# lucabaldesi/srsRAN

Hardware: AMD Instinct MI355X
Metric: PDSCH decoded Mbps + code-blocks/sec, 20 MHz TM4 QAM256, 1/2/4/8 GPU (higher is better)
Workload: dtype fp32+int16; 1 GPU; srslte_ue_dl chain from time-domain I/Q: 2048 subframes/GPU/batch, 20 MHz (100 PRB), TM4 2x2 spatial multiplexing, 2 codewords QAM256 TBS 97896 (C=16, K=6144), MMSE+CSI, max 10 half-its with CRC early stop, 40 dB crossed 2x2 channel, every subframe distinct (GPU eNodeB generator, keyed by global subframe index); 3 PHY worker threads (own ue_dl / stream / softbuffers each) decode alternate batches,; subframes_per_gpu_batch=2048, code_blocks_per_gpu_batch=65536, workers_per_gpu=3, parallelism=dp1

## Files before the change

### srsran_amd/csrc/dlsch_internal.h

```cpp
#pragma once
#include <hip/hip_runtime.h>
#include <stdint.h>

#define SB_STRIDE 18600
#define SB_DATA 768
#define SB_CONV8 10240
#define SB_ROWMASK 18544
#define SB_ROWMASK_WORDS 12

namespace mi355 {

struct CbDesc {
  uint32_t tb, cb, C;
  uint32_t rlen;
  uint32_t rp, n_e;
  uint32_t rv;
  uint32_t slot;
  uint64_t e_off;
  uint64_t data_off;
};

struct TbDesc {
  uint32_t tbs, C, C1, K1, K2, slot0, invalid;
  uint32_t Qm, nof_e_bits, rv;
// ... 98 lines not shown
```

### srsran_amd/csrc/dlsch_runtime.cpp

```cpp
#include <hip/hip_runtime.h>

#include <algorithm>
#include <chrono>
#include <stdlib.h>
#include <map>
#include <mutex>
#include <stdio.h>
#include <string.h>
#include <vector>

#include "../../include/srsran_amd/dlsch.h"
#include "../../include/srsran_amd/tdec.h"
#include "device_mem.h"
#include "dlsch_internal.h"
#include "host_staging.h"
#include "tdec8_internal.h"
#include "rm_image.h"
#include "rm_tables.h"
#include "runtime_internal.h"
#include "tdec_internal.h"

using namespace mi355;

struct mi355_softbuffer_pool {
  int      device = 0;
  uint32_t nof_sb = 0, max_cb = 0;
  int16_t* buf    = nullptr;
  uint8_t* cb_crc = nullptr;
  uint8_t* data   = nullptr;
  uint8_t* fresh  = nullptr;
  mi355::DevMem d_list[2];
  uint32_t   list_cap[2] = {0, 0};
  hipEvent_t ev_list[2]  = {nullptr, nullptr};
  bool       ev_armed[2] = {false, false};
  uint32_t   lpar        = 0;
  mi355::HostStaging st_list;
};

CrcTable mi355::make_crc_table(uint32_t poly)
{
  CrcTable t{};
  t.poly = poly;
  for (uint32_t i = 0; i < 256; i++) {
    uint32_t c = i << 16;
    for (int j = 0; j < 8; j++) c = (c & 0x800000) ? ((c << 1) ^ poly) & 0xffffff : (c << 1) & 0xffffff;
// ... 81 lines not shown
  return old;
}

static bool spec_enabled()
{
  static const bool on = !getenv("MI355_TDEC_SPEC") || atoi(getenv("MI355_TDEC_SPEC")) != 0;
  return on;
}

static bool no_rowmask()
{
  static const bool off = getenv("MI355_NO_ROWMASK") && atoi(getenv("MI355_NO_ROWMASK")) != 0;
  return off;
}

static bool lat_waves4()
{
  static const bool on = getenv("MI355_LAT_WAVES") && atoi(getenv("MI355_LAT_WAVES")) == 4;
  return on;
}
static bool lat_owaves()
{
  static const bool on = !getenv("MI355_LAT_OWAVES") || atoi(getenv("MI355_LAT_OWAVES")) != 0;
  return on;
}

bool mi355::rm_sparse_writes()
{
  static const bool on = !getenv("MI355_RM_SPARSE") || atoi(getenv("MI355_RM_SPARSE")) != 0;
  return on && !no_rowmask();
// ... 116 lines not shown
extern "C" {

int mi355_softbuffer_pool_create(mi355_softbuffer_pool_t** p, uint32_t nof_sb, uint32_t max_cb, int device)
{
  if (!p || !nof_sb || !max_cb) return MI355_ERROR_INVALID_INPUTS;
  CHECK_HIP(hipSetDevice(device));
  auto*        s  = new mi355_softbuffer_pool;
  const size_t nc = (size_t)nof_sb * max_cb;
  s->device       = device;
  s->nof_sb       = nof_sb;
  s->max_cb       = max_cb;
  if (hipMalloc(&s->buf, nc * SB_STRIDE * 2) != hipSuccess || hipMalloc(&s->cb_crc, nc) != hipSuccess ||
      hipMalloc(&s->data, nc * SB_DATA) != hipSuccess || hipMalloc(&s->fresh, nc) != hipSuccess) {
    mi355_softbuffer_pool_destroy(s);
    return MI355_ERROR;
  }
  (void)hipMemset(s->fresh, 1, nc);
  (void)hipMemset(s->cb_crc, 0, nc);
  (void)hipMemset(s->data, 0, nc * SB_DATA);
  (void)hipDeviceSynchronize();
  *p = s;
  return MI355_SUCCESS;
}

void mi355_softbuffer_pool_destroy(mi355_softbuffer_pool_t* p)
{
  if (!p) return;
  (void)hipFree(p->buf);
  (void)hipFree(p->cb_crc);
  (void)hipFree(p->data);
// ... 305 lines not shown
    }
    memcpy(all.data() + off, qlist.data(), qlist.size() * 4);
    CHECK_HIP(ent.d.upload(all));
    ent.nq = (uint32_t)qlist.size(), ent.qoff = off;
    return MI355_SUCCESS;
  });
  if (e) return e;
  *tab  = c->d.as<uint16_t>();
  *nq   = c->nq;
  *qoff = c->qoff;
  return MI355_SUCCESS;
}

mi355::SoftbufferView mi355::softbuffer_view(mi355_softbuffer_pool_t* p)
{
  return SoftbufferView{p->buf, SB_STRIDE, p->cb_crc, p->fresh, p->nof_sb, p->max_cb};
}

int mi355::dlsch_decode_dev_hook(mi355_dlsch_t* q, mi355_softbuffer_pool_t* pool, const void* d_e_bits,
                                 const mi355_dlsch_tb_t* tbs, uint32_t ntb, uint8_t* d_data, int32_t* ret,
                                 float* avg_iterations, void* stream, mi355::WaitHook hook, bool llr8,
                                 mi355::DlschPending* pend, bool after_s, bool rm_done)
{
  if (!q || !pool || !tbs || !ret || (ntb && !d_e_bits)) return MI355_ERROR_INVALID_INPUTS;
  if (ntb == 0) return MI355_SUCCESS;
  std::lock_guard<std::mutex> lock(q->mu);
  static const bool prof = getenv("MI355_HOST_PROF") != nullptr;
  auto              now  = [] { return std::chrono::steady_clock::now(); };
  const auto        t0   = now();
  CHECK_HIP(hipSetDevice(q->device));
  hipStream_t s = stream ? (hipStream_t)stream : q->own;

  std::vector<TbDesc>                        tbd(ntb);
  std::vector<std::pair<uint32_t, uint32_t>> kcount;
  std::vector<uint32_t>                      rvmask;
  std::vector<uint32_t>                      fold2;
  auto group_of = [&](uint32_t K) {
// ... 227 lines not shown
      if (lat[li]) continue;
      if (lv.t8) {
        T8Batch b{};
        b.in = (int8_t*)pool->buf, b.in_stride = SB_STRIDE * sizeof(int16_t), b.slot = d_slot + lv.off;
        b.done = d_done + lv.off, b.running = d_run + h, b.K = lv.K, b.ncb = lv.n;
        if ((r = tdec8_halfit_batch(lv.t8, b, h, lv.dec, lv.K / 8, s))) return r;
      }
      DlschCheckArgs ca{d_cb + lv.off, (int)lv.n, lv.K, h, q->max_its, lv.dec, lv.K / 8, d_data,
                        d_done + lv.off, d_run + h, d_run + h + 1, d_its + lv.off, pool->cb_crc, &crc[0], &crc[1],
                        lv.scale};
      bool fused = false;
      if (!lv.t8) {
        TdecRun rq{llr8 ? pool->buf + SB_CONV8 : pool->buf, SB_STRIDE, d_slot + lv.off, d_done + lv.off, d_run + h, lv.n,
                   lv.K, h, h + 1, lv.dec, lv.K / 8, s, &ca, &fused};
        rq.rowmask = !llr8 && !no_rowmask();
        bool taken = false;
        rq.spec       = spec;
        rq.spec_taken = &taken;
        if ((r = mi355_tdec_run_internal(lv.td, rq))) return r;
        if (!fused) CHECK_HIP(dlsch_launch_check(ca, s));
        if (taken && h + 1 < q->max_its) {
          TdecRun rd = rq;
          rd.remaining  = d_run + h + 1;
          rd.chk        = nullptr;
          rd.chk_fused  = nullptr;
          rd.spec       = false;
          rd.spec_taken = nullptr;
          rd.redo       = true;
          if ((r = mi355_tdec_run_internal(lv.td, rd))) return r;
        }
// ... 52 lines not shown
```

### srsran_amd/csrc/pdsch_internal.h

```cpp
#pragma once
#include <hip/hip_runtime.h>
#include <stdint.h>

namespace mi355 {

constexpr uint32_t EQ_BLOCK_ITEMS = 1024;

constexpr uint32_t PDSCH_GOLD_MAX = 14u * 12u * 110u * 8u;

struct PdschJobDev {
  const float2*   y[2];
  const float2*   h[4][2];
  const uint16_t* map;
  const uint16_t* imap;
  uint32_t        g0;
  float2*         d[2];
  float*          csi[2];
  uint32_t*       cmax;
  uint32_t        cmax_stride;
  uint32_t        nof_re, nof_rx, nof_ports, nof_layers, scheme, cb;
  uint32_t        row;
  uint32_t        row_magic;
  uint32_t        h_invariant;
  uint32_t        rhob_mask;
// ... 40 lines not shown
};
struct EqRmJob {
  uint32_t  C, Qm, Gp;
  EqRmLayer layer[2];
  const uint16_t* cmp[2][2];
  uint32_t        cnq[2][2], cqoff[2][2];
};
struct EqRmPool {
  int16_t*       sb;
  size_t         sb_stride;
  const uint8_t* sb_crc;
  uint8_t*       fresh;
  int            sparse;
  int            diag = 0;
  unsigned long long* prof = nullptr;
};
hipError_t pdsch_launch_eq_rm(const PdschJobDev* jobs, const EqRmJob* rj, uint32_t njobs, uint32_t max_c, uint32_t img,
                              uint32_t cimg, const uint32_t* keys, uint32_t nkeys, const EqRmPool& pool, hipStream_t s);

}
```

### srsran_amd/csrc/pdsch_kernels.hip

```cpp
#include <hip/hip_runtime.h>

#include <algorithm>
#include <stdint.h>

#include "pdsch_internal.h"
#include "rm_image.h"
#include "xcd.h"

namespace mi355 {

namespace {

struct cf {
  float re, im;
};
__device__ __forceinline__ cf mk(float r, float i) { return cf{r, i}; }
__device__ __forceinline__ cf operator+(cf a, cf b) { return mk(a.re + b.re, a.im + b.im); }
__device__ __forceinline__ cf operator-(cf a, cf b) { return mk(a.re - b.re, a.im - b.im); }
__device__ __forceinline__ cf operator*(cf a, cf b) { return mk(a.re * b.re - a.im * b.im, a.re * b.im + a.im * b.re); }
__device__ __forceinline__ cf operator*(cf a, float s) { return mk(a.re * s, a.im * s); }
__device__ __forceinline__ cf cj(cf a) { return mk(a.re, -a.im); }
__device__ __forceinline__ cf mulj(cf a) { return mk(-a.im, a.re); }
__device__ __forceinline__ float abs2(cf a) { return a.re * a.re + a.im * a.im; }
#define GLB __attribute__((address_space(1)))
// ... 1127 lines not shown
  static_assert(ER_THREADS >= 128 && 2 * (2 * SB_ROWMASK_WORDS + 1) <= 64, "pdsch_eq_rm prologue waves");
  if (tid - 64 < 2 && J.cw[tid - 64]) {
    const uint32_t l = tid - 64;
    cwd[l]           = *J.cw[l];
    cmb[l]           = cwd[l].csi_enable ? *gptr(cwd[l].cmax_final) : 0u;
  }
  __syncthreads();
  const uint32_t kx0 = c < R.layer[0].C1 ? 0u : 1u, kx1 = c < R.layer[1].C1 ? 0u : 1u;
  const bool     lean = need[0] && need[1] && fresh[0] && fresh[1] && R.layer[0].inv[kx0] == R.layer[1].inv[kx1] &&
                    R.layer[0].buflen[kx0] == R.layer[1].buflen[kx1];
  const uint32_t ev = c > R.C - gamma ? 1u : 0u;
  const bool     cm = lean && P.sparse && QM0 == QM1 && R.cmp[kx0][ev] != nullptr;
  const GLB uint16_t* fw  = cm ? gptr(R.cmp[kx0][ev]) : nullptr;
  const uint32_t      cnq = cm ? R.cnq[kx0][ev] : 0u;
  uint32_t* const     im32 = (uint32_t*)imgs;
  const unsigned long long pt1 = P.prof ? clock64() : 0ull;
  const float         noise = J.noise_dev ? *gptr(J.noise_dev) : J.noise;
  const uint32_t      row = J.row, magic = J.row_magic, rmask = J.rhob_mask;
  const float         rinv = J.rhob_inv;
  const GLB float2*   yp[2] = {gptr(J.y[0]), gptr(J.nof_rx > 1 ? J.y[1] : J.y[0])};
  const GLB float2*   hp[4];
  h_ptrs(J, hp);
  const GLB fv4*      wtp = (const GLB fv4*)gptr(J.wtab);
  uint4 iv0[ER_Q];
  if constexpr (ER_TPF) {
    if (lean) {
      const uint32_t  npairs = R.layer[0].buflen[kx0] / 2;
      const GLB uint32_t* inv32 = (const GLB uint32_t*)gptr(R.layer[0].inv[kx0]);
#pragma unroll
      for (int k = 0; k < ER_Q; k++) {
// ... 141 lines not shown
          for (int p = 0; p < 8; p++) w[p] = (m >> p) & 1u ? w[p] : 0u;
          const uint4    v0 = make_uint4(__builtin_amdgcn_perm(w[1], w[0], 0x05040100u), __builtin_amdgcn_perm(w[3], w[2], 0x05040100u),
                                         __builtin_amdgcn_perm(w[5], w[4], 0x05040100u), __builtin_amdgcn_perm(w[7], w[6], 0x05040100u));
          const uint4    v1 = make_uint4(__builtin_amdgcn_perm(w[1], w[0], 0x07060302u), __builtin_amdgcn_perm(w[3], w[2], 0x07060302u),
                                         __builtin_amdgcn_perm(w[5], w[4], 0x07060302u), __builtin_amdgcn_perm(w[7], w[6], 0x07060302u));
          const uint32_t i  = 4 * (qd[k] & 0xffffu);
          if (al && i + 3 < npairs) {
            __builtin_nontemporal_store((u4v){v0.x, v0.y, v0.z, v0.w}, (GLB u4v*)(sb[0] + i));
            __builtin_nontemporal_store((u4v){v1.x, v1.y, v1.z, v1.w}, (GLB u4v*)(sb[1] + i));
          } else {
            const uint32_t a0[4] = {v0.x, v0.y, v0.z, v0.w}, a1[4] = {v1.x, v1.y, v1.z, v1.w};
#pragma unroll
            for (int cc = 0; cc < 4; cc++)
              if (i + cc < npairs) sb[0][i + cc] = a0[cc], sb[1][i + cc] = a1[cc];
          }
        }
      }
      need[0] = need[1] = false;
    } else if (lean) {
      const uint32_t  npairs = R.layer[0].buflen[kx0] / 2, Kc = (R.layer[0].N[kx0] - 12) / 3;
      const GLB uint32_t* inv32 = (const GLB uint32_t*)gptr(R.layer[0].inv[kx0]);
      GLB uint32_t*   sb[2]  = {(GLB uint32_t*)gptr(P.sb + (size_t)slot[0] * P.sb_stride),
                                (GLB uint32_t*)gptr(P.sb + (size_t)slot[1] * P.sb_stride)};
      const bool      al     = (((uintptr_t)sb[0] | (uintptr_t)sb[1]) & 15) == 0;
      const uint16_t* a0     = (const uint16_t*)imgs;
      const uint16_t* a1     = (const uint16_t*)(imgs + img);
#pragma unroll 1
      for (int rd = 0; rd < ER_R; rd++) {
        uint4 iv[ER_Q];
#pragma unroll
        for (int k = 0; k < ER_Q; k++) {
// ... 241 lines not shown
```

### srsran_amd/csrc/pdsch_runtime.cpp

```cpp
#include <hip/hip_runtime.h>

#include <algorithm>
#include <chrono>
#include <stdlib.h>
#include <cmath>
#include <map>
#include <unordered_map>
#include <atomic>
#include <mutex>
#include <stdio.h>
#include <string.h>
#include <string>
#include <vector>

#include "../../include/srsran_amd/dlsch.h"
#include "../../include/srsran_amd/pdsch.h"
#include "../../include/srsran_amd/tdec.h"
#include "device_mem.h"
#include "host_staging.h"
#include "lte_common.h"
#include "pdsch_internal.h"
#include "rm_tables.h"
#include "runtime_internal.h"

// ... 756 lines not shown
        }
      }
    }
    if (nt < 2) {
      for (auto& row : R.cmp) row[0] = row[1] = nullptr;
    } else {
      er.cimg = std::max(er.cimg, cimg);
    }
    er.max_c = std::max(er.max_c, nt ? R.C : 0u);
    er.img   = std::max(er.img, n_max);
  }
  er.pool = EqRmPool{v.buf, v.stride, v.cb_crc, v.fresh, rm_sparse_writes() ? 1 : 0};
  static const int eqrm_diag = getenv("MI355_EQRM_DIAG") ? atoi(getenv("MI355_EQRM_DIAG")) : 0;
  er.pool.diag = eqrm_diag;
  er.pool.prof = g_eqrm_prof.load();
  return er.max_c > 0;
}

int mi355::pdsch_decode_batch_dev_noise(mi355_pdsch_t* q, mi355_softbuffer_pool_t* pool, const mi355_pdsch_job_t* jobs,
                                        uint32_t njobs, mi355_pdsch_res_t* res, void* stream, const float* d_noise,
                                        WaitHook hook, bool ce_invariant, PdschPending* pend, bool after_s)
{
  if (!q || !pool || !res || (njobs && !jobs)) return MI355_ERROR_INVALID_INPUTS;
  std::lock_guard<std::mutex> lock(q->mu);
  static const bool prof = getenv("MI355_HOST_PROF") != nullptr;
  auto              now  = [] { return std::chrono::steady_clock::now(); };
  const auto        t0   = now();
  CHECK_HIP(hipSetDevice(q->device));
  hipStream_t          s = stream ? (hipStream_t)stream : q->own;
  std::vector<JobPlan> plans(njobs);
// ... 51 lines not shown
      const uint32_t g = pend->used;
      if (pend->groups.size() <= g) {
        pend->groups.emplace_back(new DlschPending);
        pend->ret.emplace_back();
        pend->avg.emplace_back();
        pend->who.emplace_back();
      }
      dp = pend->groups[g].get(), ret = &pend->ret[g], avg = &pend->avg[g];
      pend->who[g] = by_its[its];
    }
    ret->assign(kv.second.size(), 0);
    avg->assign(kv.second.size(), 0.f);
    if ((r = mi355_dlsch_set_max_iterations(q->dlsch, its))) return r;
    const bool after = after_s || (pend && pend->used > 0);
    r = dlsch_decode_dev_hook(q->dlsch, pool, q->e_arena, kv.second.data(), (uint32_t)kv.second.size(), nullptr,
                              ret->data(), avg->data(), s, hook, q->llr8, dp, after, eqrm);
    hook = WaitHook{};
    if (r) return r;
    if (pend)
      pend->used++;
    else
      fill_results(res, by_its[its], *ret, *avg);
  }
  return MI355_SUCCESS;
}

int mi355::PdschPending::collect()
{
  int r = MI355_SUCCESS;
  for (uint32_t g = 0; g < used; g++) {
    const int e = groups[g]->collect();
// ... 12 lines not shown
```

### srsran_amd/csrc/runtime_internal.h

```cpp
#pragma once
#include "../../include/srsran_amd/dlsch.h"
#include "../../include/srsran_amd/pdsch.h"

#include <hip/hip_runtime.h>

#include <memory>
#include <utility>
#include <atomic>
#include <vector>

namespace mi355 {

struct WaitHook {
  void (*fn)(void*) = nullptr;
  void* ctx         = nullptr;
};

struct DlschPending {
  char*                host = nullptr;
  size_t               cap  = 0;
  hipEvent_t           ev   = nullptr;
  bool                 armed = false;
  uint32_t             ntb   = 0;
  size_t               avg_off = 0;
  std::vector<uint8_t> invalid;
  int32_t*             ret = nullptr;
  float*               avg = nullptr;
  std::atomic<uint32_t>* spec_mask = nullptr;
  uint32_t             max_its   = 0;
  DlschPending()                    = default;
  DlschPending(const DlschPending&) = delete;
  ~DlschPending();
  int collect();
};

int dlsch_decode_dev_hook(mi355_dlsch_t* q, mi355_softbuffer_pool_t* pool, const void* d_e_bits,
                          const mi355_dlsch_tb_t* tbs, uint32_t ntb, uint8_t* d_data, int32_t* ret, float* avg_iterations,
                          void* stream, WaitHook hook, bool llr8 = false, DlschPending* pend = nullptr,
                          bool after_s = false, bool rm_done = false);

int      dlsch_rm_inv(mi355_dlsch_t* q, uint32_t K, uint32_t rv, const uint16_t** out);
uint32_t dlsch_rm_buflen(uint32_t K);
int      dlsch_rm_compact(mi355_dlsch_t* q, uint32_t K, uint32_t rv, uint32_t E, const uint16_t** tab, uint32_t* nq,
                          uint32_t* qoff);
bool     rm_sparse_writes();
struct SoftbufferView {
  int16_t* buf;
  size_t   stride;
  uint8_t* cb_crc;
  uint8_t* fresh;
  uint32_t nof_sb, max_cb;
};
SoftbufferView softbuffer_view(mi355_softbuffer_pool_t* p);

struct PdschPending {
  std::vector<std::unique_ptr<DlschPending>>                   groups;
  std::vector<std::vector<int32_t>>                            ret;
  std::vector<std::vector<float>>                              avg;
  std::vector<std::vector<std::pair<uint32_t, uint32_t>>>      who;
  uint32_t                                                     used = 0;
  mi355_pdsch_res_t*                                           res  = nullptr;
  int collect();
};

int pdsch_decode_batch_dev_noise(mi355_pdsch_t* q, mi355_softbuffer_pool_t* pool, const mi355_pdsch_job_t* jobs,
                                 uint32_t njobs, mi355_pdsch_res_t* res, void* stream, const float* d_noise,
// ... 5 lines not shown
```

### srsran_amd/csrc/tdec_internal.h

```cpp
#pragma once
#include <hip/hip_runtime.h>
#include <stdint.h>

#include "dlsch_internal.h"

#define TDEC_INF 10000
#define TDEC_WARMUP 40
#define TDEC_SEG 8

namespace mi355 {

struct TdecWinArgs {
  const int16_t*  in;
  size_t          in_stride;
  const uint32_t* in_idx;
  const uint8_t*  done;
  const uint32_t* remaining;
  uint32_t*       A1;
  uint32_t*       E;
  uint32_t*       D;
  uint32_t*       ckpt;
  const uint32_t* dstE;
  const uint32_t* dstA;
  int             ncb, L, Lp, nseg, n, write_d;
  uint8_t*        dec;
  size_t          dec_stride;
  const uint32_t* gS;
  const uint32_t* gP;
  DlschCheckArgs  chk;
  int             chk_on;
  int             spec;
  int             rowmask;
};

struct TdecDecideArgs {
  const uint32_t* D;
  uint8_t*        out;
  size_t          out_stride;
  int             ncb, L, Lp;
  const uint8_t*  done;
  const uint32_t* remaining;
};

struct TdecGenArgs {
  const uint32_t* S;
  const uint32_t* P0;
  const uint32_t* P1;
// ... 57 lines not shown
  const int16_t*  in;
  size_t          in_stride;
  const uint32_t* in_idx;
  const uint8_t*  done;
  const uint32_t* remaining;
  uint32_t        n, K, h0, h1;
  uint8_t*        out;
  size_t          out_stride;
  hipStream_t     stream;
  const DlschCheckArgs* chk = nullptr;
  bool*                 chk_fused = nullptr;
  bool  spec       = false;
  bool* spec_taken = nullptr;
  bool  redo       = false;
  bool  rowmask    = false;
};

hipError_t tdec_win_launch_halfit(int nsb, const TdecWinArgs& a, hipStream_t s);
bool       tdec_win_spec_ok(int nsb, int L);
int        tdec_set_diag(int mode);
hipError_t tdec_win_launch_decide(int nsb, const TdecDecideArgs& a, hipStream_t s);
hipError_t tdec_gen_launch_prep(const TdecGenPrepArgs& a, hipStream_t s);
hipError_t tdec_gen_launch_halfit(const TdecGenArgs& a, hipStream_t s);
hipError_t tdec_gen_launch_decide(const TdecGenDecideArgs& a, hipStream_t s);

}

struct mi355_tdec_batch;
int mi355_tdec_run_internal(mi355_tdec_batch* q, const mi355::TdecRun& r);
int mi355_tdec_win_tables(mi355_tdec_batch* q, uint32_t K, const uint32_t** dstE, const uint32_t** dstA);
// ... 1 lines not shown
```

### srsran_amd/csrc/tdec_kernels.hip

```cpp
#include <hip/hip_runtime.h>

#include <atomic>
#include <stdint.h>
#include <stdlib.h>

#include "crc_device.h"
#include "tdec_internal.h"

namespace mi355 {

typedef short v2s __attribute__((ext_vector_type(2)));

__device__ __forceinline__ v2s U(uint32_t u) { return __builtin_bit_cast(v2s, u); }
__device__ __forceinline__ uint32_t W(v2s v) { return __builtin_bit_cast(uint32_t, v); }
__device__ __forceinline__ v2s sadd(v2s a, v2s b) { return __builtin_elementwise_add_sat(a, b); }
__device__ __forceinline__ v2s ssub(v2s a, v2s b) { return __builtin_elementwise_sub_sat(a, b); }
__device__ __forceinline__ v2s vmax(v2s a, v2s b) { return __builtin_elementwise_max(a, b); }
__device__ __forceinline__ v2s splat(short s) { return (v2s){s, s}; }
__device__ __forceinline__ uint32_t hi_lo(uint32_t a, uint32_t b) { return __builtin_amdgcn_alignbit(b, a, 16); }
__device__ __forceinline__ uint32_t from_prev(uint32_t v)
{
  return (uint32_t)__builtin_amdgcn_update_dpp(0, (int)v, 0x111, 0xf, 0xf, true);
}
__device__ __forceinline__ uint32_t from_next(uint32_t v)
// ... 110 lines not shown
      } else {
        c.done[cb] = 2;
      }
    }
  }
  const uint64_t un = __builtin_amdgcn_ballot_w64(l == 0 && !fin);
  if (un && (threadIdx.x & 63) == (uint32_t)__builtin_ctzll(un)) flag_set(c.next);
}


#define WG_AT(arr, j) (arr)[((size_t)grp * Lp + (j)) * 64 + q]

#define TDEC_BM_WORDS (8 * 193)
__shared__ uint32_t tdec_tx_lds[4][2][TDEC_SEG * 64];
__shared__ uint32_t tdec_ym_lds[4][8 * SB_ROWMASK_WORDS];
__shared__ uint32_t tdec_bm_lds[4 * TDEC_BM_WORDS];
__shared__ int16_t  tdec_stg_lds[4][TDEC_SEG * 128];
__shared__ uint32_t tdec_stg_row[4][TDEC_SEG];

#ifndef TDEC_WAVES_PER_EU
#define TDEC_WAVES_PER_EU 2
#endif
#ifndef TDEC_NPH
#define TDEC_NPH 1
#endif
#ifndef TDEC_FPF
#define TDEC_FPF 2
#endif
#ifndef TDEC_CLONE_NO_E
#define TDEC_CLONE_NO_E 0
// ... 19 lines not shown
#ifndef TDEC_OUT_AUX
#define TDEC_OUT_AUX -1
#endif
#ifndef TDEC_CK_AUX
#define TDEC_CK_AUX -1
#endif
#ifndef TDEC_CLONE_NO_FIN
#define TDEC_CLONE_NO_FIN 0
#endif
#ifndef TDEC_CLONE_NO_TAB
#define TDEC_CLONE_NO_TAB 0
#endif
#ifndef TDEC_CLONE_CK_HALF
#define TDEC_CLONE_CK_HALF 0
#endif
template <int NSB, int SEG, int MODE, int DIAG, bool FULL, int OUTK, bool GI = false, bool TX = false>
__device__ __forceinline__ void tdec_win_body(const TdecWinArgs& a, const int gl,
                                              const uint32_t (*crc_t4)[4][256] = nullptr)
{
  constexpr int NL = NSB / 2;
  constexpr int G  = 64 / NL;
  static_assert(!TX || (NSB == 16 && FULL && SEG == 8), "TX loads need 8-lane rows and whole 8-step segments");
  const int     grp = __builtin_amdgcn_readfirstlane(gl >> 6), q = gl & 63;
  const int     cbg = q / NL, l = q % NL;
  if constexpr (!TX) {
    if (grp * G + cbg >= a.ncb) return;
    if (a.done && a.done[grp * G + cbg]) return;
  }
  if (a.remaining && *a.remaining == 0) return;

  const int  L = a.L, Lp = a.Lp, nseg = a.nseg;
  constexpr bool CL     = DIAG == 20;
  constexpr bool dec2   = MODE == 2;
  constexpr bool has_ap = MODE == 1;

  const int       cb   = grp * G + cbg;
  const int       K    = L * NSB;
// ... 22 lines not shown
  }
  constexpr bool RMK = NSB == 16 && !GI;
  uint32_t*      ymask = nullptr;
  if constexpr (RMK) {
    ymask = tdec_ym_lds[threadIdx.x >> 6];
#pragma unroll
    for (int w = l; w < SB_ROWMASK_WORDS; w += NL) {
      uint32_t v = 0xffffffffu;
      if (a.rowmask) v = ((const uint32_t*)(a.in + bidx * a.in_stride + SB_ROWMASK))[(dec2 ? SB_ROWMASK_WORDS : 0) + w];
      ymask[cbg * SB_ROWMASK_WORDS + w] = v;
    }
    __builtin_amdgcn_fence(__ATOMIC_RELEASE, "wavefront");
    __builtin_amdgcn_wave_barrier();
    __builtin_amdgcn_fence(__ATOMIC_ACQUIRE, "wavefront");
  }
  auto yrow = [&](int c, int j) -> bool {
    if constexpr (RMK) {
      return (ymask[c * SB_ROWMASK_WORDS + (j >> 5)] >> (j & 31)) & 1u;
    } else {
      return true;
    }
  };
  auto tx_load = [&](int so, int j0, uint32_t* r, bool par = false) {
    uint4 v0 = make_uint4(0u, 0u, 0u, 0u), v1 = v0;
    const int tc = (q >> 1) & 7, jr = j0 + (q >> 4);
    if (!par || yrow(tc, jr)) v0 = txin[so + j0 * 2];
    if (!par || yrow(tc, jr + 4)) v1 = txin[so + (j0 + 4) * 2];
    r[0] = v0.x; r[1] = v0.y; r[2] = v0.z; r[3] = v0.w;
    r[4] = v1.x; r[5] = v1.y; r[6] = v1.z; r[7] = v1.w;
  };
  auto tx_unpack = [&](int b, const uint32_t* r, uint32_t* o) {
    uint32_t* w = txb + b * SEG * 64;
    ((uint4*)w)[q]      = make_uint4(r[0], r[1], r[2], r[3]);
    ((uint4*)w)[64 + q] = make_uint4(r[4], r[5], r[6], r[7]);
    __builtin_amdgcn_fence(__ATOMIC_RELEASE, "wavefront");
    __builtin_amdgcn_wave_barrier();
    __builtin_amdgcn_fence(__ATOMIC_ACQUIRE, "wavefront");
#pragma unroll
    for (int i = 0; i < SEG; i++) o[i] = w[64 * i + q];
  };

  v2s st[8], nw[8], aw[8];

  set_minf(aw);
#pragma unroll 1
  for (int b = 0; b < TDEC_WARMUP / 8; b++) {
    uint32_t xo[8], yo[8], ao[8] = {};
#pragma unroll
    for (int i = 0; i < 8; i++) {
      const int j = (L - TDEC_WARMUP) + 8 * b + i;
      xo[i]       = X[j * xs];
      yo[i]       = yrow(cbg, j) ? Y[j * ys] : 0u;
      if constexpr (has_ap) ao[i] = AP[j * 64];
    }
#pragma unroll
    for (int i = 0; i < 8; i++) {
      const int k = 8 * b + i;
      v2s       x = U(hi_lo(from_prev(xo[i]), xo[i]));
      if constexpr (has_ap) x = sadd(x, U(hi_lo(from_prev(ao[i]), ao[i])));
      if constexpr (CL) {
        aw[k & 7] = aw[k & 7] ^ x ^ U(yo[i]);
        continue;
      }
      v2s c0[8], c1[8];
      alpha_cands<true>(aw, x, U(hi_lo(from_prev(yo[i]), yo[i])), c0, c1);
#pragma unroll
      for (int s = 0; s < 8; s++) aw[s] = vmax(c0[s], c1[s]);
      if ((k & 1) == 0 && k != 0) normalize<true>(aw);
    }
  }

  if constexpr (DIAG != 2) {
  set_minf(st);
#pragma unroll 1
  for (int b = TDEC_WARMUP / 8 - 1; b >= 0; b--) {
    uint32_t xo[8], yo[8], ao[8] = {};
#pragma unroll
    for (int i = 0; i < 8; i++) {
      const int j = 8 * b + i;
      xo[i]       = X[j * xs];
      yo[i]       = yrow(cbg, j) ? Y[j * ys] : 0u;
      if constexpr (has_ap) ao[i] = AP[j * 64];
    }
#pragma unroll
    for (int i = 7; i >= 0; i--) {
      const int k = 8 * b + i;
      v2s       x = U(hi_lo(xo[i], from_next(xo[i])));
      if constexpr (has_ap) x = sadd(x, U(hi_lo(ao[i], from_next(ao[i]))));
      if constexpr (CL) {
        st[k & 7] = st[k & 7] ^ x ^ U(yo[i]);
        continue;
      }
      beta_step<true>(st, x, U(hi_lo(yo[i], from_next(yo[i]))), nw);
#pragma unroll
      for (int s = 0; s < 8; s++) st[s] = nw[s];
      if ((k & 1) == 0 && k != 0) normalize<true>(st);
// ... 22 lines not shown
      ck[((size_t)(nseg - 1) * 8 + s) * 64] = W(st[s]);
    }
  }

  {
    uint32_t cx[SEG], cy[SEG], ca[SEG] = {};
    auto     load = [&](int t, uint32_t* x, uint32_t* y, uint32_t* ap) {
      if constexpr (TX) {
        if constexpr (!dec2) tx_load(txoX, t * SEG, x);
        tx_load(txoY, t * SEG, y, true);
      }
#pragma unroll
      for (int i = 0; i < SEG; i++) {
        const int j = FULL ? t * SEG + i : min(t * SEG + i, L - 1);
        if constexpr (!TX || dec2) x[i] = X[j * xs];
        if constexpr (!TX) y[i] = yrow(cbg, j) ? Y[j * ys] : 0u;
        if constexpr (has_ap) ap[i] = AP[j * 64];
      }
    };
    uint32_t bx[SEG], by[SEG], ba[SEG] = {}, dx[SEG], dy[SEG], da[SEG] = {};
    load(nseg - 1, cx, cy, ca);
    if (nseg > 1) load(nseg - 2, bx, by, ba);
    auto seg = [&](int t, const uint32_t* rx, const uint32_t* ry, const uint32_t* sa, uint32_t* lx, uint32_t* ly,
                   uint32_t* la) {
      uint32_t sx[SEG], sy[SEG];
      if constexpr (TX) {
        if constexpr (!dec2) tx_unpack(0, rx, sx);
        tx_unpack(1, ry, sy);
      }
#pragma unroll
      for (int i = 0; i < SEG; i++) {
// ... 134 lines not shown
  };
  uint32_t cx[SEG], cy[SEG], ca[SEG] = {}, cd[SEG], cc[8];
  constexpr bool NFIN = CL && TDEC_CLONE_NO_FIN, NTAB = CL && TDEC_CLONE_NO_TAB, NCK = CL && TDEC_CLONE_NO_CK;
  auto     load = [&](int t, uint32_t* x, uint32_t* y, uint32_t* ap, uint32_t* d, uint32_t* c) {
    if constexpr (TX && !NFIN) {
      if constexpr (!dec2) tx_load(txoX, t * SEG, x);
      tx_load(txoY, t * SEG, y, true);
    }
#pragma unroll
    for (int i = 0; i < SEG; i++) {
      const int j = FULL ? t * SEG + i : min(t * SEG + i, L - 1);
      if constexpr (NFIN) {
        x[i] = y[i] = (uint32_t)j;
      } else {
        if constexpr (!TX || dec2) x[i] = Xf[j * xs];
        if constexpr (!TX) y[i] = yrow(cbg, j) ? Yf[j * ys] : 0u;
      }
      if constexpr (has_ap) ap[i] = APf[j * 64];
      if constexpr (NTAB) {
        d[i] = (uint32_t)(j * 128 + 2 * l) | ((uint32_t)(j * 128 + 2 * l + 1) << 16);
      } else {
        d[i] = tab[(size_t)j * NL];
      }
    }
#pragma unroll
    for (int s = 0; s < 8; s++) {
      c[s] = (NCK || (CL && TDEC_CLONE_CK_HALF && (t & 1))) ? (uint32_t)s : ckf[((size_t)t * 8 + s) * 64];
    }
  };
  load(0, cx, cy, ca, cd, cc);

// ... 183 lines not shown
      crc_t4[1][0][ti] = a.chk.crc24b->t[ti];
      __syncthreads();
#pragma unroll
      for (int k = 1; k < 4; k++) {
        crc_t4[0][k][ti] = crc24_step_table(crc_t4[0][k - 1][ti], crc_t4[0][0]);
        crc_t4[1][k][ti] = crc24_step_table(crc_t4[1][k - 1][ti], crc_t4[1][0]);
        __syncthreads();
      }
      t4 = crc_t4;
    }
  }
  if constexpr (TX) {
    const int  cb  = (gl >> 6) * (128 / NSB) + (gl & 63) / (NSB / 2);
    const bool act = cb < a.ncb && !(a.done && a.done[cb]);
    if (__builtin_amdgcn_ballot_w64(act) == ~0ull) {
      tdec_win_body<NSB, SEG, MODE, DIAG, FULL, OUTK, false, true>(a, gl, t4);
      return;
    }
  }
  tdec_win_body<NSB, SEG, MODE, DIAG, FULL, OUTK>(a, gl, t4);
}


template <int NSB>
__global__ __launch_bounds__(256) void tdec_win_decide_rows(TdecDecideArgs a)
{
  constexpr int NL = NSB / 2;
  constexpr int G  = 64 / NL;
  const size_t  g  = (size_t)blockIdx.x * blockDim.x + threadIdx.x;
  const int     q  = (int)(g & 63);
// ... 175 lines not shown
```

### srsran_amd/csrc/tdec_runtime.cpp

```cpp
#include <hip/hip_runtime.h>

#include <map>
#include <mutex>
#include <stdio.h>
#include <string.h>
#include <vector>

#include "../../include/srsran_amd/tdec.h"
#include "device_mem.h"
#include "lte_qpp_table.h"
#include "tdec_internal.h"

using namespace mi355;

namespace {

int cb_index(uint32_t K)
{
  for (int i = 0; i < LTE_NOF_CB_SIZES; i++) {
    if (lte_qpp_table[i][0] == K) return i;
    if (lte_qpp_table[i][0] > K) break;
  }
  return -1;
}
// ... 225 lines not shown
    const size_t arr = (size_t)g.ngrp * g.Lp * 64 * 4;
    static const size_t pad = getenv("MI355_TDEC_WS_PAD") ? (size_t)atoll(getenv("MI355_TDEC_WS_PAD")) : 0;
    auto*        A1  = (uint32_t*)carve(arr + pad);
    auto*        E   = (uint32_t*)carve(arr + pad);
    auto*        D   = (uint32_t*)carve(arr + pad);
    auto*        CK  = (uint32_t*)carve((size_t)g.ngrp * g.nseg * 8 * 64 * 4);

    const bool fuse = (g.L % 8 == 0 || (K % 64 == 0 && (K / 8) % (g.nsb / 2) == 0)) && out_stride % 8 == 0 &&
                      (uintptr_t)d_out % 8 == 0;
    const uint32_t *dstE = t->dstE.as<uint32_t>(), *dstA = t->dstA.as<uint32_t>();
    for (uint32_t h = h0; h < h1; h++) {
      if (rq.redo) {
        TdecWinArgs wa{d_in, in_stride, rq.in_idx, rq.done, rq.remaining, A1, E, D, CK, dstE, dstA,
                       (int)n, (int)g.L, (int)g.Lp, (int)g.nseg, (int)h, 0, nullptr, out_stride};
        wa.rowmask = rq.rowmask && g.nsb == 16 && in_stride == SB_STRIDE;
        CHECK_HIP(tdec_win_launch_halfit(g.nsb, wa, s));
        continue;
      }
      TdecWinArgs wa{d_in, in_stride, rq.in_idx, rq.done, rq.remaining, A1, E, D, CK, dstE, dstA,
                     (int)n, (int)g.L, (int)g.Lp, (int)g.nseg, (int)h, h + 1 == h1,
                     (fuse && h + 1 == h1) ? d_out : nullptr, out_stride};
      wa.rowmask = rq.rowmask && g.nsb == 16 && in_stride == SB_STRIDE;
      if (rq.spec && fuse && h + 1 == h1 && tdec_win_spec_ok(g.nsb, g.L)) {
        wa.spec = 1;
        if (rq.spec_taken) *rq.spec_taken = true;
      }
      if (rq.chk && fuse && h + 1 == h1) {
        wa.chk    = *rq.chk;
        wa.chk.h  = h;
        wa.chk_on = 1;
        if (rq.chk_fused) *rq.chk_fused = true;
      }
      hipEvent_t e0 = nullptr, e1 = nullptr;
      if (q->prof) {
        e0 = next_event(q);
        e1 = next_event(q);
        if (e0) (void)hipEventRecord(e0, s);
// ... 233 lines not shown
```

Baseline: 126,600 Mbps.

## Write compacted parity side image in eq/RM and read it in turbo decoder

The fused equalizer/rate-dematching kernel now also writes the parity rows that the row mask marks as present into a compact per-slot side buffer. It tags each softbuffer with a serial number. When the tag matches, the turbo decoder reads parity from this dense buffer using popcount ranks instead of doing strided sparse reads from the full softbuffer. This is meant to cut scattered memory traffic for the parity streams, at the cost of an extra allocation, extra nontemporal stores, and rank bookkeeping in LDS.

```diff
diff --git a/srsran_amd/csrc/dlsch_internal.h b/srsran_amd/csrc/dlsch_internal.h
--- a/srsran_amd/csrc/dlsch_internal.h
+++ b/srsran_amd/csrc/dlsch_internal.h
@@ -7,6 +7,10 @@
 #define SB_CONV8 10240
 #define SB_ROWMASK 18544
 #define SB_ROWMASK_WORDS 12
+#define PAR_SIDE_ROWS 96
+#define PAR_SIDE_STREAM (PAR_SIDE_ROWS * 32)
+#define PAR_SIDE_SLOT (2 * PAR_SIDE_STREAM)
+#define SB_PARTAG (2 * SB_ROWMASK_WORDS + 1)
 
 namespace mi355 {
 
diff --git a/srsran_amd/csrc/dlsch_runtime.cpp b/srsran_amd/csrc/dlsch_runtime.cpp
--- a/srsran_amd/csrc/dlsch_runtime.cpp
+++ b/srsran_amd/csrc/dlsch_runtime.cpp
@@ -29,6 +29,7 @@
   uint8_t* cb_crc = nullptr;
   uint8_t* data   = nullptr;
   uint8_t* fresh  = nullptr;
+  mi355::DevMem side;
   mi355::DevMem d_list[2];
   uint32_t   list_cap[2] = {0, 0};
   hipEvent_t ev_list[2]  = {nullptr, nullptr};
@@ -140,6 +141,21 @@
   return off;
 }
 
+static bool no_parside()
+{
+  const char* e = getenv("MI355_NO_PARSIDE");
+  return e && atoi(e) != 0;
+}
+
+uint32_t mi355::parside_next_serial()
+{
+  static std::atomic<uint32_t> next{0};
+  uint32_t                     v;
+  do v = next.fetch_add(1u) + 1u;
+  while (v == 0);
+  return v;
+}
+
 static bool lat_waves4()
 {
   static const bool on = getenv("MI355_LAT_WAVES") && atoi(getenv("MI355_LAT_WAVES")) == 4;
@@ -286,6 +302,13 @@
       hipMalloc(&s->data, nc * SB_DATA) != hipSuccess || hipMalloc(&s->fresh, nc) != hipSuccess) {
     mi355_softbuffer_pool_destroy(s);
     return MI355_ERROR;
+  }
+  if (!no_parside() && !no_rowmask() && nc * PAR_SIDE_SLOT < ((size_t)1 << 31)) {
+    if (s->side.alloc(nc * PAR_SIDE_SLOT) != hipSuccess ||
+        hipMemset2D(s->buf + SB_ROWMASK + 2 * SB_PARTAG, SB_STRIDE * 2, 0, 8, nc) != hipSuccess) {
+      mi355_softbuffer_pool_destroy(s);
+      return MI355_ERROR;
+    }
   }
   (void)hipMemset(s->fresh, 1, nc);
   (void)hipMemset(s->cb_crc, 0, nc);
@@ -621,13 +644,13 @@
 
 mi355::SoftbufferView mi355::softbuffer_view(mi355_softbuffer_pool_t* p)
 {
-  return SoftbufferView{p->buf, SB_STRIDE, p->cb_crc, p->fresh, p->nof_sb, p->max_cb};
+  return SoftbufferView{p->buf, SB_STRIDE, p->cb_crc, p->fresh, p->nof_sb, p->max_cb, p->side.as<int16_t>()};
 }
 
 int mi355::dlsch_decode_dev_hook(mi355_dlsch_t* q, mi355_softbuffer_pool_t* pool, const void* d_e_bits,
                                  const mi355_dlsch_tb_t* tbs, uint32_t ntb, uint8_t* d_data, int32_t* ret,
                                  float* avg_iterations, void* stream, mi355::WaitHook hook, bool llr8,
-                                 mi355::DlschPending* pend, bool after_s, bool rm_done)
+                                 mi355::DlschPending* pend, bool after_s, bool rm_done, uint32_t par_serial)
 {
   if (!q || !pool || !tbs || !ret || (ntb && !d_e_bits)) return MI355_ERROR_INVALID_INPUTS;
   if (ntb == 0) return MI355_SUCCESS;
@@ -885,6 +908,11 @@
         TdecRun rq{llr8 ? pool->buf + SB_CONV8 : pool->buf, SB_STRIDE, d_slot + lv.off, d_done + lv.off, d_run + h, lv.n,
                    lv.K, h, h + 1, lv.dec, lv.K / 8, s, &ca, &fused};
         rq.rowmask = !llr8 && !no_rowmask();
+        if (rq.rowmask && rm_done && par_serial && pool->side.p) {
+          rq.par        = pool->side.as<int16_t>();
+          rq.par_bytes  = (uint32_t)pool->side.bytes;
+          rq.par_serial = par_serial;
+        }
         bool taken = false;
         rq.spec       = spec;
         rq.spec_taken = &taken;
diff --git a/srsran_amd/csrc/pdsch_internal.h b/srsran_amd/csrc/pdsch_internal.h
--- a/srsran_amd/csrc/pdsch_internal.h
+++ b/srsran_amd/csrc/pdsch_internal.h
@@ -78,6 +78,8 @@
   int            sparse;
   int            diag = 0;
   unsigned long long* prof = nullptr;
+  int16_t* side   = nullptr;
+  uint32_t serial = 0;
 };
 hipError_t pdsch_launch_eq_rm(const PdschJobDev* jobs, const EqRmJob* rj, uint32_t njobs, uint32_t max_c, uint32_t img,
                               uint32_t cimg, const uint32_t* keys, uint32_t nkeys, const EqRmPool& pool, hipStream_t s);
diff --git a/srsran_amd/csrc/pdsch_kernels.hip b/srsran_amd/csrc/pdsch_kernels.hip
--- a/srsran_amd/csrc/pdsch_kernels.hip
+++ b/srsran_amd/csrc/pdsch_kernels.hip
@@ -1165,6 +1165,22 @@
   const GLB uint16_t* fw  = cm ? gptr(R.cmp[kx0][ev]) : nullptr;
   const uint32_t      cnq = cm ? R.cnq[kx0][ev] : 0u;
   uint32_t* const     im32 = (uint32_t*)imgs;
+  __shared__ uint32_t prk[2 * SB_ROWMASK_WORDS];
+  __shared__ uint32_t puse[2];
+  const uint32_t      Kcm  = (R.layer[0].N[kx0] - 12) / 3;
+  const bool          side = cm && P.side != nullptr && Kcm > 800 && Kcm % 16 == 0;
+  if (side && tid < 2 * SB_ROWMASK_WORDS) {
+    const uint32_t s = tid / SB_ROWMASK_WORDS, w = tid % SB_ROWMASK_WORDS, L = Kcm / 16;
+    uint32_t       pre = 0, tot = 0;
+    for (uint32_t k = 0; k < SB_ROWMASK_WORDS; k++) {
+      const uint32_t rows = L > 32 * k ? min(32u, L - 32 * k) : 0u;
+      const uint32_t n    = __popc(nbm[0][s * SB_ROWMASK_WORDS + k] & (rows == 32 ? 0xffffffffu : (1u << rows) - 1u));
+      pre += k < w ? n : 0u;
+      tot += n;
+    }
+    prk[tid] = pre;
+    if (w == 0) puse[s] = tot <= PAR_SIDE_ROWS && L <= 32 * SB_ROWMASK_WORDS ? 1u : 0u;
+  }
   const unsigned long long pt1 = P.prof ? clock64() : 0ull;
   const float         noise = J.noise_dev ? *gptr(J.noise_dev) : J.noise;
   const uint32_t      row = J.row, magic = J.row_magic, rmask = J.rhob_mask;
@@ -1336,7 +1352,26 @@
             for (int cc = 0; cc < 4; cc++)
               if (i + cc < npairs) sb[0][i + cc] = a0[cc], sb[1][i + cc] = a1[cc];
           }
-        }
+          if (side) {
+            const uint32_t pos = 2 * i, sl = Kcm + 32;
+            const uint32_t st  = (pos >= sl ? 1u : 0u) + (pos >= 2 * sl ? 1u : 0u) + (pos >= 3 * sl ? 1u : 0u);
+            const uint32_t ps  = st - 1, j = (pos - st * sl) >> 4;
+            if ((st == 1 || st == 2) && j < Kcm / 16 && puse[ps]) {
+              const uint32_t wd = nbm[0][ps * SB_ROWMASK_WORDS + (j >> 5)];
+              const uint32_t rk = prk[ps * SB_ROWMASK_WORDS + (j >> 5)] + __popc(wd & ((1u << (j & 31)) - 1u));
+              if (((wd >> (j & 31)) & 1u) && rk < PAR_SIDE_ROWS) {
+                const size_t o = ps * (PAR_SIDE_STREAM / 2) + rk * 16 + ((pos - st * sl) & 8u);
+                __builtin_nontemporal_store((u4v){v0.x, v0.y, v0.z, v0.w},
+                                            (GLB u4v*)gptr(P.side + (size_t)slot[0] * (PAR_SIDE_SLOT / 2) + o));
+                __builtin_nontemporal_store((u4v){v1.x, v1.y, v1.z, v1.w},
+                                            (GLB u4v*)gptr(P.side + (size_t)slot[1] * (PAR_SIDE_SLOT / 2) + o));
+              }
+            }
+          }
+        }
+      }
+      if (side && tid < 4) {
+        rm_rowmask_of(P.sb + (size_t)slot[tid >> 1] * P.sb_stride)[SB_PARTAG + (tid & 1)] = puse[tid & 1] ? P.serial : 0u;
       }
       need[0] = need[1] = false;
     } else if (lean) {
diff --git a/srsran_amd/csrc/pdsch_runtime.cpp b/srsran_amd/csrc/pdsch_runtime.cpp
--- a/srsran_amd/csrc/pdsch_runtime.cpp
+++ b/srsran_amd/csrc/pdsch_runtime.cpp
@@ -794,6 +794,10 @@
   static const int eqrm_diag = getenv("MI355_EQRM_DIAG") ? atoi(getenv("MI355_EQRM_DIAG")) : 0;
   er.pool.diag = eqrm_diag;
   er.pool.prof = g_eqrm_prof.load();
+  if (v.side && er.pool.sparse) {
+    er.pool.side   = v.side;
+    er.pool.serial = parside_next_serial();
+  }
   return er.max_c > 0;
 }
 
@@ -875,7 +879,7 @@
     if ((r = mi355_dlsch_set_max_iterations(q->dlsch, its))) return r;
     const bool after = after_s || (pend && pend->used > 0);
     r = dlsch_decode_dev_hook(q->dlsch, pool, q->e_arena, kv.second.data(), (uint32_t)kv.second.size(), nullptr,
-                              ret->data(), avg->data(), s, hook, q->llr8, dp, after, eqrm);
+                              ret->data(), avg->data(), s, hook, q->llr8, dp, after, eqrm, eqrm ? er.pool.serial : 0u);
     hook = WaitHook{};
     if (r) return r;
     if (pend)
diff --git a/srsran_amd/csrc/runtime_internal.h b/srsran_amd/csrc/runtime_internal.h
--- a/srsran_amd/csrc/runtime_internal.h
+++ b/srsran_amd/csrc/runtime_internal.h
@@ -37,7 +37,8 @@
 int dlsch_decode_dev_hook(mi355_dlsch_t* q, mi355_softbuffer_pool_t* pool, const void* d_e_bits,
                           const mi355_dlsch_tb_t* tbs, uint32_t ntb, uint8_t* d_data, int32_t* ret, float* avg_iterations,
                           void* stream, WaitHook hook, bool llr8 = false, DlschPending* pend = nullptr,
-                          bool after_s = false, bool rm_done = false);
+                          bool after_s = false, bool rm_done = false, uint32_t par_serial = 0);
+uint32_t parside_next_serial();
 
 int      dlsch_rm_inv(mi355_dlsch_t* q, uint32_t K, uint32_t rv, const uint16_t** out);
 uint32_t dlsch_rm_buflen(uint32_t K);
@@ -50,6 +51,7 @@
   uint8_t* cb_crc;
   uint8_t* fresh;
   uint32_t nof_sb, max_cb;
+  int16_t* side;
 };
 SoftbufferView softbuffer_view(mi355_softbuffer_pool_t* p);
 
diff --git a/srsran_amd/csrc/tdec_internal.h b/srsran_amd/csrc/tdec_internal.h
--- a/srsran_amd/csrc/tdec_internal.h
+++ b/srsran_amd/csrc/tdec_internal.h
@@ -31,6 +31,8 @@
   int             chk_on;
   int             spec;
   int             rowmask;
+  const int16_t*  par;
+  uint32_t        par_bytes, par_serial;
 };
 
 struct TdecDecideArgs {
@@ -118,6 +120,8 @@
   bool* spec_taken = nullptr;
   bool  redo       = false;
   bool  rowmask    = false;
+  const int16_t* par = nullptr;
+  uint32_t       par_bytes = 0, par_serial = 0;
 };
 
 hipError_t tdec_win_launch_halfit(int nsb, const TdecWinArgs& a, hipStream_t s);
diff --git a/srsran_amd/csrc/tdec_kernels.hip b/srsran_amd/csrc/tdec_kernels.hip
--- a/srsran_amd/csrc/tdec_kernels.hip
+++ b/srsran_amd/csrc/tdec_kernels.hip
@@ -148,6 +148,7 @@
 #define TDEC_BM_WORDS (8 * 193)
 __shared__ uint32_t tdec_tx_lds[4][2][TDEC_SEG * 64];
 __shared__ uint32_t tdec_ym_lds[4][8 * SB_ROWMASK_WORDS];
+__shared__ uint32_t tdec_yr_lds[4][8 * SB_ROWMASK_WORDS];
 __shared__ uint32_t tdec_bm_lds[4 * TDEC_BM_WORDS];
 __shared__ int16_t  tdec_stg_lds[4][TDEC_SEG * 128];
 __shared__ uint32_t tdec_stg_row[4][TDEC_SEG];
@@ -197,13 +198,14 @@
 #ifndef TDEC_CLONE_CK_HALF
 #define TDEC_CLONE_CK_HALF 0
 #endif
-template <int NSB, int SEG, int MODE, int DIAG, bool FULL, int OUTK, bool GI = false, bool TX = false>
+template <int NSB, int SEG, int MODE, int DIAG, bool FULL, int OUTK, bool GI = false, bool TX = false, bool PS = false>
 __device__ __forceinline__ void tdec_win_body(const TdecWinArgs& a, const int gl,
                                               const uint32_t (*crc_t4)[4][256] = nullptr)
 {
   constexpr int NL = NSB / 2;
   constexpr int G  = 64 / NL;
   static_assert(!TX || (NSB == 16 && FULL && SEG == 8), "TX loads need 8-lane rows and whole 8-step segments");
+  static_assert(!PS || (TX && !GI && DIAG == 0), "side-image waves are TX waves of the product kernel");
   const int     grp = __builtin_amdgcn_readfirstlane(gl >> 6), q = gl & 63;
   const int     cbg = q / NL, l = q % NL;
   if constexpr (!TX) {
@@ -256,6 +258,31 @@
     __builtin_amdgcn_wave_barrier();
     __builtin_amdgcn_fence(__ATOMIC_ACQUIRE, "wavefront");
   }
+  constexpr bool  PSR   = RMK && !TX && DIAG == 0;
+  bool            ytag  = false;
+  const uint32_t* YS    = Y;
+  uint32_t*       yrank = nullptr;
+  if constexpr (PS || PSR) {
+    yrank = tdec_yr_lds[threadIdx.x >> 6];
+    if constexpr (PS) {
+      ytag = true;
+    } else if (a.par && a.rowmask) {
+      ytag = ((const uint32_t*)(a.in + bidx * a.in_stride + SB_ROWMASK))[SB_PARTAG + (dec2 ? 1 : 0)] == a.par_serial;
+    }
+    if (ytag) {
+      YS = (const uint32_t*)(a.par + bidx * (PAR_SIDE_SLOT / 2) + (dec2 ? PAR_SIDE_STREAM / 2 : 0)) + l;
+#pragma unroll
+      for (int w = l; w < SB_ROWMASK_WORDS; w += NL) {
+        uint32_t pre = 0;
+#pragma unroll
+        for (int k = 0; k < SB_ROWMASK_WORDS; k++) pre += k < w ? __popc(ymask[cbg * SB_ROWMASK_WORDS + k]) : 0;
+        yrank[cbg * SB_ROWMASK_WORDS + w] = pre;
+      }
+    }
+    __builtin_amdgcn_fence(__ATOMIC_RELEASE, "wavefront");
+    __builtin_amdgcn_wave_barrier();
+    __builtin_amdgcn_fence(__ATOMIC_ACQUIRE, "wavefront");
+  }
   auto yrow = [&](int c, int j) -> bool {
     if constexpr (RMK) {
       return (ymask[c * SB_ROWMASK_WORDS + (j >> 5)] >> (j & 31)) & 1u;
@@ -263,9 +290,49 @@
       return true;
     }
   };
+  auto yld = [&](const uint32_t* Yp, int j) -> uint32_t {
+    if constexpr (PS || PSR) {
+      const uint32_t m = ymask[cbg * SB_ROWMASK_WORDS + (j >> 5)], b = (uint32_t)j & 31u;
+      if (!((m >> b) & 1u)) return 0u;
+      const uint32_t* p = Yp + j * ys;
+      if (ytag) {
+        const uint32_t rk = yrank[cbg * SB_ROWMASK_WORDS + (j >> 5)] + __popc(m & ((1u << b) - 1u));
+        p                 = YS + min(rk, (uint32_t)PAR_SIDE_ROWS - 1u) * NL;
+      }
+      return *p;
+    } else {
+      return yrow(cbg, j) ? Yp[j * ys] : 0u;
+    }
+  };
+  [[maybe_unused]] const __amdgpu_buffer_rsrc_t psr =
+      __builtin_amdgcn_make_buffer_rsrc((void*)a.par, 0, PS ? (int)a.par_bytes : 0, 0x00020000);
+  [[maybe_unused]] uint32_t pbase = 0, pm = 0, pp = 0;
+  [[maybe_unused]] int      pw = -1;
+  if constexpr (PS) {
+    const int txc = grp * G + ((q >> 1) & 7);
+    pbase = a.in_idx[txc] * (uint32_t)PAR_SIDE_SLOT + (dec2 ? (uint32_t)PAR_SIDE_STREAM : 0u) + 16u * (q & 1);
+  }
   auto tx_load = [&](int so, int j0, uint32_t* r, bool par = false) {
     uint4 v0 = make_uint4(0u, 0u, 0u, 0u), v1 = v0;
     const int tc = (q >> 1) & 7, jr = j0 + (q >> 4);
+    if constexpr (PS) {
+      if (par) {
+        if ((j0 >> 5) != pw) {
+          pw = j0 >> 5;
+          pm = ymask[tc * SB_ROWMASK_WORDS + pw];
+          pp = yrank[tc * SB_ROWMASK_WORDS + pw];
+        }
+        typedef uint32_t u4v __attribute__((ext_vector_type(4)));
+        const uint32_t b0 = (uint32_t)jr & 31u, b1 = b0 + 4u;
+        const uint32_t o0 = (pm >> b0) & 1u ? pbase + 32u * (pp + __popc(pm & ((1u << b0) - 1u))) : 0x80000000u;
+        const uint32_t o1 = (pm >> b1) & 1u ? pbase + 32u * (pp + __popc(pm & ((1u << b1) - 1u))) : 0x80000000u;
+        const u4v      w0 = __builtin_amdgcn_raw_buffer_load_b128(psr, (int)o0, 0, 0);
+        const u4v      w1 = __builtin_amdgcn_raw_buffer_load_b128(psr, (int)o1, 0, 0);
+        r[0] = w0.x; r[1] = w0.y; r[2] = w0.z; r[3] = w0.w;
+        r[4] = w1.x; r[5] = w1.y; r[6] = w1.z; r[7] = w1.w;
+        return;
+      }
+    }
     if (!par || yrow(tc, jr)) v0 = txin[so + j0 * 2];
     if (!par || yrow(tc, jr + 4)) v1 = txin[so + (j0 + 4) * 2];
     r[0] = v0.x; r[1] = v0.y; r[2] = v0.z; r[3] = v0.w;
@@ -292,7 +359,7 @@
     for (int i = 0; i < 8; i++) {
       const int j = (L - TDEC_WARMUP) + 8 * b + i;
       xo[i]       = X[j * xs];
-      yo[i]       = yrow(cbg, j) ? Y[j * ys] : 0u;
+      yo[i]       = yld(Y, j);
       if constexpr (has_ap) ao[i] = AP[j * 64];
     }
 #pragma unroll
@@ -321,7 +388,7 @@
     for (int i = 0; i < 8; i++) {
       const int j = 8 * b + i;
       xo[i]       = X[j * xs];
-      yo[i]       = yrow(cbg, j) ? Y[j * ys] : 0u;
+      yo[i]       = yld(Y, j);
       if constexpr (has_ap) ao[i] = AP[j * 64];
     }
 #pragma unroll
@@ -374,7 +441,7 @@
       for (int i = 0; i < SEG; i++) {
         const int j = FULL ? t * SEG + i : min(t * SEG + i, L - 1);
         if constexpr (!TX || dec2) x[i] = X[j * xs];
-        if constexpr (!TX) y[i] = yrow(cbg, j) ? Y[j * ys] : 0u;
+        if constexpr (!TX) y[i] = yld(Y, j);
         if constexpr (has_ap) ap[i] = AP[j * 64];
       }
     };
@@ -539,7 +606,7 @@
         x[i] = y[i] = (uint32_t)j;
       } else {
         if constexpr (!TX || dec2) x[i] = Xf[j * xs];
-        if constexpr (!TX) y[i] = yrow(cbg, j) ? Yf[j * ys] : 0u;
+        if constexpr (!TX) y[i] = yld(Yf, j);
       }
       if constexpr (has_ap) ap[i] = APf[j * 64];
       if constexpr (NTAB) {
@@ -753,6 +820,15 @@
     const int  cb  = (gl >> 6) * (128 / NSB) + (gl & 63) / (NSB / 2);
     const bool act = cb < a.ncb && !(a.done && a.done[cb]);
     if (__builtin_amdgcn_ballot_w64(act) == ~0ull) {
+      if constexpr (DIAG == 0) {
+        if (a.par && a.rowmask && a.in_idx) {
+          const uint32_t* bmw = (const uint32_t*)(a.in + (size_t)a.in_idx[cb] * a.in_stride + SB_ROWMASK);
+          if (__builtin_amdgcn_ballot_w64(bmw[SB_PARTAG + (MODE == 2 ? 1 : 0)] == a.par_serial) == ~0ull) {
+            tdec_win_body<NSB, SEG, MODE, DIAG, FULL, OUTK, false, true, true>(a, gl, t4);
+            return;
+          }
+        }
+      }
       tdec_win_body<NSB, SEG, MODE, DIAG, FULL, OUTK, false, true>(a, gl, t4);
       return;
     }
diff --git a/srsran_amd/csrc/tdec_runtime.cpp b/srsran_amd/csrc/tdec_runtime.cpp
--- a/srsran_amd/csrc/tdec_runtime.cpp
+++ b/srsran_amd/csrc/tdec_runtime.cpp
@@ -263,6 +263,7 @@
         TdecWinArgs wa{d_in, in_stride, rq.in_idx, rq.done, rq.remaining, A1, E, D, CK, dstE, dstA,
                        (int)n, (int)g.L, (int)g.Lp, (int)g.nseg, (int)h, 0, nullptr, out_stride};
         wa.rowmask = rq.rowmask && g.nsb == 16 && in_stride == SB_STRIDE;
+        if (wa.rowmask && rq.in_idx) wa.par = rq.par, wa.par_bytes = rq.par_bytes, wa.par_serial = rq.par_serial;
         CHECK_HIP(tdec_win_launch_halfit(g.nsb, wa, s));
         continue;
       }
@@ -270,6 +271,7 @@
                      (int)n, (int)g.L, (int)g.Lp, (int)g.nseg, (int)h, h + 1 == h1,
                      (fuse && h + 1 == h1) ? d_out : nullptr, out_stride};
       wa.rowmask = rq.rowmask && g.nsb == 16 && in_stride == SB_STRIDE;
+      if (wa.rowmask && rq.in_idx) wa.par = rq.par, wa.par_bytes = rq.par_bytes, wa.par_serial = rq.par_serial;
       if (rq.spec && fuse && h + 1 == h1 && tdec_win_spec_ok(g.nsb, g.L)) {
         wa.spec = 1;
         if (rq.spec_taken) *rq.spec_taken = true;
```

Result: no change. 126,400 Mbps, median of 2 (-0.2%).
